# slimgroup/SetIntersectionProjection.jl

Measured on AMD Instinct MI355X. Metric: PARSDMM iterations/sec, higher is better.
Workload: dtype f32

## Files before the change

### setintersectionprojection.jl_amd/csrc/kernels_cds.hip

```cpp
#include <cstdlib>
#include <stdexcept>
#include <string>

#include "sipx_device.h"
#define SIPX_CG_GRID launch_blocks(3)
#ifndef SIPX_F64_VEC
#define SIPX_F64_VEC 2
#endif

namespace sipx {

template <typename T, int V>
struct LoadStored {
  const T* __restrict__ x;
  __device__ __forceinline__ Vec<T, V> operator()(long long c) const { return ldv_u<T, V>(x + c); }
};
template <typename T, int V>
struct LoadFused {
  const T* __restrict__ r;
  const T* __restrict__ p;
  T beta;
  __device__ __forceinline__ Vec<T, V> operator()(long long c) const {
    const Vec<T, V> rv = ldv_u<T, V>(r + c), pv = ldv_u<T, V>(p + c);
    Vec<T, V> o;
#pragma unroll
    for (int k = 0; k < V; ++k) o.v[k] = rv.v[k] + beta * pv.v[k];
    return o;
  }
};

template <typename T, int V, int D, typename XL>
__device__ __forceinline__ void cds_rows(long long N, const T* __restrict__ R, const CdsArgs& a, const XL& xl, long long r,
                                         T (&acc)[V]) {
  const int d = D ? D : a.d;
#pragma unroll
  for (int k = 0; k < V; ++k) acc[k] = T(0);
  if constexpr (D > 0) {
    Vec<T, V> rv[D], xv[D];
#pragma unroll
    for (int b = 0; b < D; ++b) {
      if (a.sym) {
        rv[b] = a.off[b] >= 0 ? ldv<T, V>(R + (long long)b * N + r)
                              : ldv_u<T, V>(R + (long long)a.partner[b] * N + r + a.off[b]);
      } else {
        rv[b] = ldv_nt<T, V>(R + (long long)b * N + r);
      }
      xv[b] = xl(r + a.off[b]);
    }
#pragma unroll
    for (int b = 0; b < D; ++b) {
      const long long c = r + a.off[b];
#pragma unroll
      for (int k = 0; k < V; ++k) {
        const T t = acc[k] + rv[b].v[k] * xv[b].v[k];
        acc[k] = (c + k >= 0 && c + k < N) ? t : acc[k];
      }
    }
  } else {
    for (int b = 0; b < d; ++b) {
      const long long c = r + a.off[b];
      const Vec<T, V> rv = !a.sym ? ldv_nt<T, V>(R + (long long)b * N + r)
                                  : (a.off[b] >= 0 ? ldv<T, V>(R + (long long)b * N + r)
                                                   : ldv_u<T, V>(R + (long long)a.partner[b] * N + c));
      const Vec<T, V> xv = xl(c);
#pragma unroll
      for (int k = 0; k < V; ++k) {
        const T t = acc[k] + rv.v[k] * xv.v[k];
        acc[k] = (c + k >= 0 && c + k < N) ? t : acc[k];
      }
    }
  }
}

template <typename T, int V, int D, int MODE>
__global__ __launch_bounds__(BLOCK) void k_cds(long long N, long long r0, long long r1, const T* __restrict__ R, CdsArgs a,
                                               const T* __restrict__ x, T* __restrict__ y, const T* __restrict__ b,
                                               T* __restrict__ pout, T* __restrict__ xold, double* __restrict__ partials,
                                               const int* __restrict__ done) {
  if (MODE == 1 && *done) return;
  const long long nvec = r1 / V;
  double acc0 = 0, acc1 = 0;
  for (long long vi = r0 / V + (long long)blockIdx.x * BLOCK + threadIdx.x; vi < nvec; vi += (long long)gridDim.x * BLOCK) {
    const long long r = vi * V;
    T s[V];
    cds_rows<T, V, D>(N, R, a, LoadStored<T, V>{x}, r, s);
    if (MODE == 0) {
      Vec<T, V> o;
#pragma unroll
      for (int k = 0; k < V; ++k) o.v[k] = s[k];
      stv_nt<T, V>(y + r, o);
    } else if (MODE == 1) {
      const Vec<T, V> pv = ldv<T, V>(x + r);
      Vec<T, V> o;
#pragma unroll
      for (int k = 0; k < V; ++k) {
        o.v[k] = s[k];
        acc0 += (double)pv.v[k] * (double)s[k];
      }
      stv_nt<T, V>(y + r, o);
    } else {
      const Vec<T, V> bv = ldv<T, V>(b + r);
      const Vec<T, V> xv = ldv<T, V>(x + r);
      Vec<T, V> o;
#pragma unroll
      for (int k = 0; k < V; ++k) {
        o.v[k] = bv.v[k] - s[k];
        acc0 += (double)o.v[k] * (double)o.v[k];
        acc1 += (double)bv.v[k] * (double)bv.v[k];
      }
      stv<T, V>(y + r, o);
      if (pout) stv<T, V>(pout + r, o);
      if (xold) stv<T, V>(xold + r, xv);
    }
  }
  if (MODE == 1) {
    double acc[1] = {acc0};
    block_reduce_store<1>(acc, partials, 0);
  } else if (MODE == 2) {
    double acc[2] = {acc0, acc1};
    block_reduce_store<2>(acc, partials, 0);
  }
}

constexpr int march_role(int ord, int b) {
  constexpr int o1[7] = {0, 1, 2, 3, 4, 5, 6}, o2[7] = {0, 5, 3, 1, 2, 4, 6};
  return ord == 1 ? o1[b] : o2[b];
}
template <typename T>
__device__ __forceinline__ T ata_value(const Grid& G, int nblk, const int* dir, const T* ihs, long long o, const Coord& c) {
  T val = (nblk == 0 && o == 0) ? T(1) : T(0);
  for (int q = 0; q < nblk; ++q) {
    const int d = dir[q];
    const T ih = ihs[q], nih = -ih;
    const int cc = coord_of(c, d);
    const long long st = G.st[d];
    if (o == 0) {
      if (cc > 0) val = val + ih * ih;
      if (cc < G.n[d] - 1) val = val + nih * nih;
    } else if (o == st) {
      if (cc < G.n[d] - 1) val = val + nih * ih;
    } else if (o == -st) {
      if (cc > 0) val = val + ih * nih;
    }
  }
  return val;
}

constexpr int QP_MAXB = 9, QP_MAXT = 8, QP_TAB = 160;
struct QPlanTerm {
  int kind;
  int nblk;
  int dir[3];
  int tab;
};
template <typename T>
struct QPlan {
  int nbands;
  int col[QP_MAXB], nterms[QP_MAXB];
  QPlanTerm t[QP_MAXB][QP_MAXT];
  int ntab;
  T tab[QP_TAB];
};

struct NoExtra {};
template <typename T>
struct QTab {
  const T* tab;
};
template <typename X>
struct IsQTab { static constexpr bool value = false; };
template <typename T>
struct IsQTab<QTab<T>> { static constexpr bool value = true; };
template <typename T>
__device__ __forceinline__ void load_class_tab(const QTab<T>& u, T* tab) {
  for (int i = threadIdx.x; i < QT_N; i += blockDim.x) tab[i] = u.tab[i];
}
template <typename X, typename T>
__device__ __forceinline__ void load_class_tab(const X&, T*) {}
__device__ __forceinline__ int line_class(long long c, long long n) { return c == 0 ? 0 : (c == n - 1 ? 2 : 1); }
template <typename T, int V>
__device__ __forceinline__ Vec<T, V> tab_row(const T* tab, int role, int cyz, long long i0, long long n1) {
  const T* e = tab + 27 * role + cyz;
  const T first = e[0], mid = e[1], last = e[2];
  Vec<T, V> v;
#pragma unroll
  for (int k = 0; k < V; ++k) v.v[k] = i0 + k == 0 ? first : (i0 + k == n1 - 1 ? last : mid);
  return v;
}
__device__ __forceinline__ void publish_ticket(unsigned long long* ticket, unsigned seq, int iter, int done);
constexpr int MARCH_NT = 512;
template <typename T, int V, int ORD, int MODE, typename X>
__global__ __launch_bounds__(MARCH_NT) void k_cds_march(long long n1, long long n2, long long n3, long long z0, long long z1, const T* __restrict__ R0,
                                                        const T* __restrict__ R1, const T* __restrict__ R2, const T* __restrict__ R3,
                                                        const T* __restrict__ x, T* __restrict__ y, const T* __restrict__ b,
                                                        T* __restrict__ pout, T* __restrict__ xold, double* __restrict__ partials,
                                                        const int* __restrict__ done, int lgLX, int tiles_x, int tiles_y, int zchunk,
                                                        long long items, CgState<T>* __restrict__ st, CgState<T>* __restrict__ host,
                                                        unsigned long long* ticket, X extra) {
  constexpr bool TAB = IsQTab<X>::value;
  if (MODE == 1 && *done) return;
  T beta = T(0);
  if (MODE == 3) {
    if (st->done) return;
    const double ss = block_sum_partials_n<MARCH_NT>(partials + NB);
    const T rr = (T)ss;
    const T res = (T)sqrt(ss) / st->nr0;
    const bool conv = res <= st->tol;
    beta = rr / st->gamma;
    if (blockIdx.x == 0 && threadIdx.x == 0) {
      st->ss = ss;
      st->res_last = res;
      if (conv) { st->flag = 0; st->done = 1; } else { st->beta = beta; }
      st->rr = rr;
      *host = *st;
      publish_ticket(ticket, st->seq, st->iters, conv ? 1 : 0);
    }
    if (conv) return;
  }
  auto ldx = [&](long long at) -> Vec<T, V> {
    Vec<T, V> v = ldv<T, V>(x + at);
    if (MODE == 3) {
      const Vec<T, V> pv = ldv<T, V>(b + at);
#pragma unroll
      for (int k = 0; k < V; ++k) v.v[k] = v.v[k] + beta * pv.v[k];
    }
    return v;
  };
  auto ldx1 = [&](long long at) -> T { return MODE == 3 ? x[at] + beta * b[at] : x[at]; };
  __shared__ T sx[2][V][MARCH_NT], sr[TAB ? 1 : 2][TAB ? 1 : V][TAB ? 1 : MARCH_NT];
  __shared__ T ctab[TAB ? QT_N : 1];
  if (TAB) {
    load_class_tab(extra, ctab);
    __syncthreads();
  }
  const int tid = threadIdx.x, LX = 1 << lgLX, tx = tid & (LX - 1), ty = tid >> lgLX, TY = MARCH_NT >> lgLX;
  const long long st1 = n1, st2 = n1 * n2, N = st2 * n3;
  const long long tiles = (long long)tiles_x * tiles_y;
  double acc0 = 0, acc1 = 0;
  for (long long item = blockIdx.x; item < items; item += gridDim.x) {
    const long long zc = item / tiles, tile = item - zc * tiles;
    const int tile_y = (int)(tile / tiles_x), tile_x = (int)(tile - (long long)tile_y * tiles_x);
    const long long i0 = ((long long)tile_x * LX + tx) * V, j = (long long)tile_y * TY + ty;
    const bool active = i0 < n1 && j < n2;
    const long long k0 = z0 + zc * zchunk, k1 = (k0 + zchunk < z1) ? k0 + zchunk : z1;
    const unsigned go = active ? (unsigned)(i0 + st1 * j) : 0u;
    __syncthreads();
    Vec<T, V> xm = zerov<T, V>(), x0 = zerov<T, V>(), rzm = zerov<T, V>();
    if (active) {
      xm = ldx(st2 * (k0 - 1) + go);
      x0 = ldx(st2 * k0 + go);
      if (k0 > 0 && TAB) {
        rzm = tab_row<T, V>(ctab, 3, 3 * line_class(j, n2) + 9 * line_class(k0 - 1, n3), i0, n1);
      } else if (k0 > 0) {
        rzm = ldv<T, V>(R3 + st2 * (k0 - 1) + go);
      }
    }
    for (long long kz = k0; kz < k1; ++kz) {
      const int par = (int)(kz & 1);
      const long long pz = st2 * kz;
      Vec<T, V> xp = zerov<T, V>(), r0 = xp, r1 = xp, r2 = xp, r3 = xp, bv = xp;
      const int cz = TAB ? line_class(kz, n3) : 0, cyz = TAB ? 3 * line_class(j, n2) + 9 * cz : 0;
      const int cyz_up = !TAB ? 0 : (j > 0 ? 3 * line_class(j - 1, n2) + 9 * cz : 3 * line_class(n2 - 1, n2) + 9 * line_class(kz - 1, n3));
      if (active) {
        xp = ldx(pz + st2 + go);
        if constexpr (TAB) {
          r0 = tab_row<T, V>(ctab, 0, cyz, i0, n1);
          r1 = tab_row<T, V>(ctab, 1, cyz, i0, n1);
          r2 = tab_row<T, V>(ctab, 2, cyz, i0, n1);
          r3 = tab_row<T, V>(ctab, 3, cyz, i0, n1);
        } else {
          r0 = ldv_nt<T, V>(R0 + pz + go);
          r1 = ldv_nt<T, V>(R1 + pz + go);
          r2 = ldv_nt<T, V>(R2 + pz + go);
          r3 = ldv_nt<T, V>(R3 + pz + go);
        }
        if (MODE == 2) bv = ldv<T, V>(b + pz + go);
      }
#pragma unroll
      for (int k = 0; k < V; ++k) {
        sx[par][k][tid] = x0.v[k];
        if constexpr (!TAB) sr[par][k][tid] = r2.v[k];
      }
      T xl = __shfl_up(x0.v[V - 1], 1, 64), xr = __shfl_down(x0.v[0], 1, 64), rl = TAB ? T(0) : __shfl_up(r1.v[V - 1], 1, 64);
      const long long r = pz + go;
      if (TAB && r > 0)
        rl = i0 > 0 ? ctab[27 + line_class(i0 - 1, n1) + cyz] : ctab[27 + line_class(n1 - 1, n1) + cyz_up];
      if (active) {
        if (tx == 0 || (tid & 63) == 0) {
          xl = ldx1(r - 1);
          if (!TAB) rl = r > 0 ? R1[r - 1] : T(0);
        }
        if (tx == LX - 1 || (tid & 63) == 63) xr = ldx1(r + V);
      }
      __syncthreads();
      if (active) {
        Vec<T, V> xu = zerov<T, V>(), xd = xu, ru = xu;
        if (TAB && r - st1 >= 0) ru = tab_row<T, V>(ctab, 2, cyz_up, i0, n1);
        if (ty > 0) {
#pragma unroll
          for (int k = 0; k < V; ++k) {
            xu.v[k] = sx[par][k][tid - LX];
            if constexpr (!TAB) ru.v[k] = sr[par][k][tid - LX];
          }
        } else {
          xu = ldx(r - st1);
          if (!TAB && r - st1 >= 0) ru = ldv<T, V>(R2 + r - st1);
        }
        if (ty < TY - 1 && j + 1 < n2) {
#pragma unroll
          for (int k = 0; k < V; ++k) xd.v[k] = sx[par][k][tid + LX];
        } else {
          xd = ldx(r + st1);
        }
        const bool up = r >= st1, down = r + st1 < N, below = r >= st2, above = r + st2 < N, first = r == 0, last = r + V == N;
        Vec<T, V> o4;
#pragma unroll
        for (int k = 0; k < V; ++k) {
          const T rv[7] = {r0.v[k], k == 0 ? rl : r1.v[k - 1], r1.v[k], ru.v[k], r2.v[k], rzm.v[k], r3.v[k]};
          const T xv[7] = {x0.v[k], k == 0 ? xl : x0.v[k - 1], k == V - 1 ? xr : x0.v[k + 1], xu.v[k], xd.v[k], xm.v[k], xp.v[k]};
          const bool in[7] = {true, k > 0 || !first, k < V - 1 || !last, up, down, below, above};
          T acc = T(0);
#pragma unroll
          for (int q = 0; q < 7; ++q) {
            const int role = march_role(ORD, q);
            const T t = acc + rv[role] * xv[role];
            acc = in[role] ? t : acc;
          }
          o4.v[k] = acc;
        }
        if (MODE == 0) {
          stv_nt<T, V>(y + r, o4);
        } else if (MODE == 1 || MODE == 3) {
#pragma unroll
          for (int k = 0; k < V; ++k) acc0 += (double)x0.v[k] * (double)o4.v[k];
          stv_nt<T, V>(y + r, o4);
          if (MODE == 3) stv<T, V>(pout + r, x0);
        } else {
          Vec<T, V> o;
#pragma unroll
          for (int k = 0; k < V; ++k) {
            o.v[k] = bv.v[k] - o4.v[k];
            acc0 += (double)o.v[k] * (double)o.v[k];
            acc1 += (double)bv.v[k] * (double)bv.v[k];
          }
          stv<T, V>(y + r, o);
          if (pout) stv<T, V>(pout + r, o);
          if (xold) stv<T, V>(xold + r, x0);
        }
      }
      xm = x0; x0 = xp; rzm = r3;
    }
  }
  if (MODE != 0) {
    __shared__ double sm[2][MARCH_NT / 64];
    const double v0 = wave_sum(acc0), v1 = wave_sum(acc1);
    __syncthreads();
    if ((tid & 63) == 0) { sm[0][tid >> 6] = v0; sm[1][tid >> 6] = v1; }
    __syncthreads();
    if (tid < (MODE == 2 ? 2 : 1)) {
      double s = 0;
#pragma unroll
      for (int i = 0; i < MARCH_NT / 64; ++i) s += sm[tid][i];
      double* row = partials + (long long)tid * NB;
      row[blockIdx.x] = s;
      for (int jj = blockIdx.x + gridDim.x; jj < NB; jj += gridDim.x) row[jj] = 0.0;
    }
  }
}

struct MarchGeom {
  int lg, tiles_x, tiles_y, zchunk, grid;
  long long items;
};
template <typename T>
static bool march_geom(long long N, long long r0, long long r1, const CdsArgs& a, MarchGeom& m) {
  const int sw = env_knobs().cds_march;
  const long long zc_env = env_knobs().cds_march_zchunk;
  if (sw == 0 || !a.march || !a.sym || a.d != 7) return false;
  constexpr int V = sizeof(T) == 8 ? 2 : 4;
  const long long n1 = a.gn[0], n2 = a.gn[1], n3 = a.gn[2], st2 = n1 * n2;
  if (n1 % V != 0 || n1 * n2 * n3 != N || r0 % st2 != 0 || r1 % st2 != 0 || r1 <= r0) return false;
  const long long nvx = n1 / V;
  int lg = 0;
  while ((1 << lg) < nvx && lg < 6) ++lg;
  const int LX = 1 << lg, TY = MARCH_NT / LX;
  const int tiles_x = (int)((nvx + LX - 1) / LX), tiles_y = (int)((n2 + TY - 1) / TY);
  const long long tiles = (long long)tiles_x * tiles_y, planes = (r1 - r0) / st2;
  long long zchunk = planes * tiles / 2048;
  if (zchunk < 16) zchunk = 16;
  if (sw == 2 && zc_env > 0) zchunk = zc_env;
  if (zchunk > planes) zchunk = planes;
  const long long nchunks = (planes + zchunk - 1) / zchunk, items = tiles * nchunks;
  if (items < 384 && sw != 2) return false;
  m = MarchGeom{lg, tiles_x, tiles_y, (int)zchunk, (int)(items < NB ? items : NB), items};
  return true;
}
template <typename T>
bool K<T>::march_applies(long long N, const CdsArgs& a) {
  MarchGeom m;
  return march_geom<T>(N, 0, N, a, m);
}

template <typename T, int MODE>
static bool try_march(hipStream_t s, long long N, long long r0, long long r1, const T* R, const CdsArgs& a, const T* x, T* y, const T* b,
                      T* pout, T* xold, double* partials, const int* done, CgState<T>* st = nullptr, CgState<T>* host = nullptr,
                      unsigned long long* ticket = nullptr) {
  MarchGeom m;
  if (!march_geom<T>(N, r0, r1, a, m)) return false;
  constexpr int V = sizeof(T) == 8 ? 2 : 4;
  const long long n1 = a.gn[0], n2 = a.gn[1], n3 = a.gn[2], st2 = n1 * n2;
  const T *R0 = R + (long long)a.mb[0] * N, *R1 = R + (long long)a.mb[1] * N, *R2 = R + (long long)a.mb[2] * N, *R3 = R + (long long)a.mb[3] * N;
#define SIPX_MARCH(ORD, XT, XV)                                                                                                      \
  hipLaunchKernelGGL((k_cds_march<T, V, ORD, MODE, XT>), dim3(m.grid), dim3(MARCH_NT), 0, s, n1, n2, n3, r0 / st2, r1 / st2, R0, R1, R2, R3, x, y, b, \
                     pout, xold, partials, done, m.lg, m.tiles_x, m.tiles_y, m.zchunk, m.items, st, host, ticket, XV)
  if (a.qtab) {
    const QTab<T> tab{(const T*)a.qtab};
    if (a.march == 1) SIPX_MARCH(1, QTab<T>, tab);
    else SIPX_MARCH(2, QTab<T>, tab);
  } else if (a.march == 1) {
    SIPX_MARCH(1, NoExtra, NoExtra{});
  } else {
    SIPX_MARCH(2, NoExtra, NoExtra{});
  }
#undef SIPX_MARCH
  return true;
}

template <typename T, int MODE>
static void launch_cds(hipStream_t s, long long N, long long r0, long long r1, const T* R, const CdsArgs& a, const T* x, T* y,
                       const T* b, T* pout, T* xold, double* partials, const int* done) {
  if (a.d < 1 || a.d > MAXD) throw std::runtime_error("cds: band count out of range");
  if (r0 < 0 || r1 > N || r0 > r1) throw std::runtime_error("cds: row range outside the matrix");
  int read_bands = a.d;
  if (a.sym) { read_bands = 0; for (int b = 0; b < a.d; ++b) read_bands += a.off[b] >= 0 ? 1 : 0; }
  if (a.qtab) read_bands = 0;
  const double rw = (double)(r1 - r0) * sizeof(T), extra = MODE == 2 ? 4.0 : 2.0;
  const double moved_extra = (MODE == 2 && !xold) ? 3.0 : extra;
  ObsScope obs(MODE == 0 ? KID_CDS_SPMV : (MODE == 1 ? KID_CDS_DOT : KID_CDS_RESID), s, (a.d + extra) * rw, (read_bands + moved_extra) * rw);
  if (try_march<T, MODE>(s, N, r0, r1, R, a, x, y, b, pout, xold, partials, done)) {
    SIPX_HIP(hipGetLastError());
    return;
  }
  if (a.qtab) throw std::runtime_error("internal: Q's class table is in use but the z-marching product does not apply");
#define SIPX_CDS(V, D) \
  hipLaunchKernelGGL((k_cds<T, V, D, MODE>), dim3(fit_grid((r1 - r0) / V, SIPX_CG_GRID)), dim3(BLOCK), 0, s, N, r0, r1, R, a, x, y, b, pout, xold, partials, done)
  constexpr int VW = sizeof(T) == 8 ? SIPX_F64_VEC : 4;
  if (N % 4 == 0 && r0 % 4 == 0 && r1 % 4 == 0) {
    switch (a.d) {
      case 1: SIPX_CDS(VW, 1); break;
      case 3: SIPX_CDS(VW, 3); break;
      case 5: SIPX_CDS(VW, 5); break;
      case 7: SIPX_CDS(VW, 7); break;
      default: SIPX_CDS(VW, 0); break;
    }
  } else {
    SIPX_CDS(1, 0);
  }
#undef SIPX_CDS
  SIPX_HIP(hipGetLastError());
}

template <typename T>
void K<T>::spmv(hipStream_t s, const Grid&, long long N, const T* R, const CdsArgs& a, const T* x, T* y) {
  launch_cds<T, 0>(s, N, 0, N, R, a, x, y, nullptr, nullptr, nullptr, nullptr, nullptr);
}
template <typename T>
void K<T>::spmv_dot(hipStream_t s, long long N, long long r0, long long r1, const T* R, const CdsArgs& a, const T* p, T* Ap,
                    double* partials, const CgState<T>* st) {
  launch_cds<T, 1>(s, N, r0, r1, R, a, p, Ap, nullptr, nullptr, nullptr, partials, &st->done);
}
template <typename T>
void K<T>::resid(hipStream_t s, long long N, long long r0, long long r1, const T* R, const CdsArgs& a, const T* x, const T* b,
                 T* r, T* p, T* xold, double* partials) {
  launch_cds<T, 2>(s, N, r0, r1, R, a, x, r, b, p, xold, partials, nullptr);
}

template <typename T, int V>
__device__ __forceinline__ void stencil_rows(const Grid& G, const StencilQ<T>& q, const T* __restrict__ x, long long g,
                                             const Vec<T, V>& xc, T (&acc)[V]) {
  const Coord c = coords(G, g);
#pragma unroll
  for (int k = 0; k < V; ++k) acc[k] = q.w0 * xc.v[k];
#pragma unroll
  for (int dir = 0; dir < 3; ++dir) {
    if (!(q.mask & (1 << dir))) continue;
    const long long st = G.st[dir];
    const int nd = (int)G.n[dir], cd = coord_of(c, dir);
    const Vec<T, V> xm = ldv_u<T, V>(x + g - st), xp = ldv_u<T, V>(x + g + st);
#pragma unroll
    for (int k = 0; k < V; ++k) {
      const int ck = cd + (dir == 0 ? k : 0);
      const T a = xc.v[k] - xm.v[k], b = xc.v[k] - xp.v[k];
      const T t = (ck > 0 ? a : T(0)) + (ck < nd - 1 ? b : T(0));
      acc[k] = acc[k] + q.w[dir] * t;
    }
  }
}

template <typename T, int V, int MODE>
__global__ __launch_bounds__(BLOCK) void k_sq(Grid G, StencilQ<T> q, const T* __restrict__ x, T* __restrict__ y,
                                              const T* __restrict__ b, T* __restrict__ pout, T* __restrict__ xold,
                                              double* __restrict__ partials, const int* __restrict__ done) {
  if (MODE == 1 && *done) return;
  const long long nvec = G.N / V;
  double acc0 = 0, acc1 = 0;
  for (long long vi = (long long)blockIdx.x * BLOCK + threadIdx.x; vi < nvec; vi += (long long)gridDim.x * BLOCK) {
    const long long r = vi * V;
    const Vec<T, V> xv = ldv<T, V>(x + r);
    T s[V];
    stencil_rows<T, V>(G, q, x, r, xv, s);
    Vec<T, V> o;
    if (MODE == 0) {
#pragma unroll
      for (int k = 0; k < V; ++k) o.v[k] = s[k];
      stv_nt<T, V>(y + r, o);
    } else if (MODE == 1) {
#pragma unroll
      for (int k = 0; k < V; ++k) {
        o.v[k] = s[k];
        acc0 += (double)xv.v[k] * (double)s[k];
      }
      stv_nt<T, V>(y + r, o);
    } else {
      const Vec<T, V> bv = ldv<T, V>(b + r);
#pragma unroll
      for (int k = 0; k < V; ++k) {
        o.v[k] = bv.v[k] - s[k];
        acc0 += (double)o.v[k] * (double)o.v[k];
        acc1 += (double)bv.v[k] * (double)bv.v[k];
      }
      stv<T, V>(y + r, o);
      if (pout) stv<T, V>(pout + r, o);
      if (xold) stv<T, V>(xold + r, xv);
    }
  }
  if (MODE == 1) {
    double acc[1] = {acc0};
    block_reduce_store<1>(acc, partials, 0);
  } else if (MODE == 2) {
    double acc[2] = {acc0, acc1};
    block_reduce_store<2>(acc, partials, 0);
  }
}

template <typename T, int MODE>
static void launch_sq(hipStream_t s, const Grid& G, const StencilQ<T>& q, const T* x, T* y, const T* b, T* pout, T* xold,
                      double* partials, const int* done) {
  ObsScope obs(MODE == 0 ? KID_SQ_SPMV : (MODE == 1 ? KID_SQ_DOT : KID_SQ_RESID), s, (MODE == 2 ? 4.0 : 2.0) * (double)G.N * sizeof(T));
  if (G.N % 4 == 0 && G.n[0] % 4 == 0)
    hipLaunchKernelGGL((k_sq<T, 4, MODE>), dim3(NB_7), dim3(BLOCK), 0, s, G, q, x, y, b, pout, xold, partials, done);
  else
    hipLaunchKernelGGL((k_sq<T, 1, MODE>), dim3(NB_7), dim3(BLOCK), 0, s, G, q, x, y, b, pout, xold, partials, done);
  SIPX_HIP(hipGetLastError());
}
template <typename T>
void K<T>::sq_spmv(hipStream_t s, const Grid& G, const StencilQ<T>& q, const T* x, T* y) {
  launch_sq<T, 0>(s, G, q, x, y, nullptr, nullptr, nullptr, nullptr, nullptr);
}
template <typename T>
void K<T>::sq_spmv_dot(hipStream_t s, const Grid& G, const StencilQ<T>& q, const T* p, T* Ap, double* partials,
                       const CgState<T>* st) {
  launch_sq<T, 1>(s, G, q, p, Ap, nullptr, nullptr, nullptr, partials, &st->done);
}
template <typename T>
void K<T>::sq_resid(hipStream_t s, const Grid& G, const StencilQ<T>& q, const T* x, const T* b, T* r, T* p, T* xold,
                    double* partials) {
  launch_sq<T, 2>(s, G, q, x, r, b, p, xold, partials, nullptr);
}

template <typename T, int V>
__global__ __launch_bounds__(BLOCK) void k_q_axpy(long long N, T* __restrict__ q, const T* __restrict__ a, T alpha) {
  const long long nvec = N / V;
  for (long long vi = (long long)blockIdx.x * BLOCK + threadIdx.x; vi < nvec; vi += (long long)gridDim.x * BLOCK) {
    Vec<T, V> qv = ldv<T, V>(q + vi * V);
    const Vec<T, V> av = ldv<T, V>(a + vi * V);
#pragma unroll
    for (int k = 0; k < V; ++k) qv.v[k] = qv.v[k] + alpha * av.v[k];
    stv<T, V>(q + vi * V, qv);
  }
}
template <typename T>
void K<T>::q_axpy(hipStream_t s, long long N, T* Qband, const T* Aband, T alpha) {
  if (N % 4 == 0)
    hipLaunchKernelGGL((k_q_axpy<T, 4>), dim3(NB), dim3(BLOCK), 0, s, N, Qband, Aband, alpha);
  else
    hipLaunchKernelGGL((k_q_axpy<T, 1>), dim3(NB), dim3(BLOCK), 0, s, N, Qband, Aband, alpha);
  SIPX_HIP(hipGetLastError());
}

struct GenArgs {
  int nblk;
  int dir[3];
  int nband;
  long long off[7];
};
template <typename T>
__global__ __launch_bounds__(BLOCK) void k_gen_ata(Grid G, GenArgs a, T ih0, T ih1, T ih2, T* __restrict__ R) {
  const T ihs[3] = {ih0, ih1, ih2};
  for (long long g = (long long)blockIdx.x * BLOCK + threadIdx.x; g < G.N; g += (long long)gridDim.x * BLOCK) {
    const Coord c = coords(G, g);
    for (int b = 0; b < a.nband; ++b) R[(long long)b * G.N + g] = ata_value<T>(G, a.nblk, a.dir, ihs, a.off[b], c);
  }
}

template <typename T, int V>
__global__ __launch_bounds__(BLOCK) void k_q_update(Grid G, long long r0, long long r1, CdsArgs q, QArgs<T> a, T* __restrict__ Q) {
  const long long nvec = r1 / V;
  for (long long vi = r0 / V + (long long)blockIdx.x * BLOCK + threadIdx.x; vi < nvec; vi += (long long)gridDim.x * BLOCK) {
    const long long g = vi * V;
    Coord c[V];
#pragma unroll
    for (int k = 0; k < V; ++k) { c[k] = coords(G, g); c[k].i += k; }
    for (int b = 0; b < q.d; ++b) {
      const long long o = q.off[b];
      if (q.sym && o < 0) continue;
      bool touched = false;
      Vec<T, V> qv;
      for (int si = 0; si < a.nsets; ++si) {
        const QSet<T>& S = a.s[si];
        int j = -1;
        for (int t = 0; t < S.nband; ++t) if (S.off[t] == o) j = t;
        if (j < 0) continue;
        if (!touched) { qv = ldv<T, V>(Q + (long long)b * G.N + g); touched = true; }
        if (S.ata) {
          const Vec<T, V> av = ldv_nt<T, V>(S.ata + (long long)j * G.N + g);
#pragma unroll
          for (int k = 0; k < V; ++k) qv.v[k] = qv.v[k] + S.alpha * av.v[k];
        } else {
#pragma unroll
          for (int k = 0; k < V; ++k) qv.v[k] = qv.v[k] + S.alpha * ata_value<T>(G, S.nblk, S.dir, S.ih, o, c[k]);
        }
      }
      if (touched) stv<T, V>(Q + (long long)b * G.N + g, qv);
    }
  }
}

template <typename T, int V>
__global__ __launch_bounds__(BLOCK) void k_q_update_plan(Grid G, long long r0, long long r1, QPlan<T> p, T* __restrict__ Q) {
  __shared__ T tab[QP_TAB];
  for (int i = threadIdx.x; i < p.ntab; i += BLOCK) tab[i] = p.tab[i];
  __syncthreads();
  const int n1 = (int)G.n[0], n2 = (int)G.n[1], n3 = (int)G.n[2];
  const long long nvec = r1 / V;
  for (long long vi = r0 / V + (long long)blockIdx.x * BLOCK + threadIdx.x; vi < nvec; vi += (long long)gridDim.x * BLOCK) {
    const long long g = vi * V;
    const Coord c = coords(G, g);
    int cx[V];
#pragma unroll
    for (int k = 0; k < V; ++k) cx[k] = (c.i + k) == 0 ? 0 : ((c.i + k) == n1 - 1 ? 2 : 1);
    const int cy = c.j == 0 ? 0 : (c.j == n2 - 1 ? 2 : 1), cz = c.k == 0 ? 0 : (c.k == n3 - 1 ? 2 : 1);
    for (int b = 0; b < p.nbands; ++b) {
      T* row = Q + (long long)p.col[b] * G.N + g;
      Vec<T, V> qv = ldv<T, V>(row);
      for (int ti = 0; ti < p.nterms[b]; ++ti) {
        const QPlanTerm& t = p.t[b][ti];
        if (t.kind == 0) {
          const T v = tab[t.tab];
#pragma unroll
          for (int k = 0; k < V; ++k) qv.v[k] = qv.v[k] + v;
        } else if (t.kind == 1) {
          int base = 0, mulx = 0, m3 = 1;
          for (int q = 0; q < t.nblk; ++q) {
            const int d = t.dir[q];
            if (d == 0) mulx += m3; else base += (d == 1 ? cy : cz) * m3;
            m3 *= 3;
          }
#pragma unroll
          for (int k = 0; k < V; ++k) qv.v[k] = qv.v[k] + tab[t.tab + base + mulx * cx[k]];
        } else {
          const int d = t.dir[0];
          const int edge = t.kind == 2 ? 2 : 0;
          const T on = tab[t.tab], off = tab[t.tab + 1];
#pragma unroll
          for (int k = 0; k < V; ++k) {
            const int cl = d == 0 ? cx[k] : (d == 1 ? cy : cz);
            qv.v[k] = qv.v[k] + (cl != edge ? on : off);
          }
        }
      }
      stv<T, V>(row, qv);
    }
  }
}
// ... 574 lines not shown
```

Before: 898.0.

## Software-pipeline next-plane loads in CDS march stencil kernel

Restructures the z-marching stencil loop so that the next plane's x, halo-edge and side loads are issued one iteration ahead and drained with an explicit s_waitcnt before the stores. Edge loads for the up, down and left/right neighbours are merged into a single precomputed offset per thread, and the pipeline depth is chosen at compile time per mode and table variant. The intent is to hide global-memory latency behind the stencil arithmetic. In exchange it raises register pressure, which the occupancy hint of 4 blocks per CU in launch_bounds may force into spills, and it adds a 32-bit offset guard on the geometry.

Measured after the change: 906.4 (median of 6 runs). Within noise of the previous version (+0.9%).

```diff
diff --git a/setintersectionprojection.jl_amd/csrc/kernels_cds.hip b/setintersectionprojection.jl_amd/csrc/kernels_cds.hip
--- a/setintersectionprojection.jl_amd/csrc/kernels_cds.hip
+++ b/setintersectionprojection.jl_amd/csrc/kernels_cds.hip
@@ -190,7 +190,7 @@
 __device__ __forceinline__ void publish_ticket(unsigned long long* ticket, unsigned seq, int iter, int done);
 constexpr int MARCH_NT = 512;
 template <typename T, int V, int ORD, int MODE, typename X>
-__global__ __launch_bounds__(MARCH_NT) void k_cds_march(long long n1, long long n2, long long n3, long long z0, long long z1, const T* __restrict__ R0,
+__global__ __launch_bounds__(MARCH_NT, 4) void k_cds_march(long long n1, long long n2, long long n3, long long z0, long long z1, const T* __restrict__ R0,
                                                         const T* __restrict__ R1, const T* __restrict__ R2, const T* __restrict__ R3,
                                                         const T* __restrict__ x, T* __restrict__ y, const T* __restrict__ b,
                                                         T* __restrict__ pout, T* __restrict__ xold, double* __restrict__ partials,
@@ -198,6 +198,8 @@
                                                         long long items, CgState<T>* __restrict__ st, CgState<T>* __restrict__ host,
                                                         unsigned long long* ticket, X extra) {
   constexpr bool TAB = IsQTab<X>::value;
+  constexpr int DEPTH = TAB ? ((MODE != 3 || sizeof(T) == 4) ? 2 : 1) : (MODE < 2 ? 2 : 0);
+  constexpr bool AHEAD = DEPTH == 2;
   if (MODE == 1 && *done) return;
   T beta = T(0);
   if (MODE == 3) {
@@ -217,16 +219,49 @@
     }
     if (conv) return;
   }
-  auto ldx = [&](long long at) -> Vec<T, V> {
-    Vec<T, V> v = ldv<T, V>(x + at);
-    if (MODE == 3) {
-      const Vec<T, V> pv = ldv<T, V>(b + at);
-#pragma unroll
-      for (int k = 0; k < V; ++k) v.v[k] = v.v[k] + beta * pv.v[k];
-    }
+  struct XRaw { Vec<T, V> a, b; };
+  struct XRaw1 { T a, b; };
+  struct PlaneRaw {
+    XRaw xp, e;
+    XRaw1 s;
+    Vec<T, V> bv;
+  };
+  struct PlaneIn {
+    Vec<T, V> xp, e;
+    T s;
+    Vec<T, V> bv;
+  };
+  auto ldraw = [&](long long at) -> XRaw {
+    XRaw v;
+    v.a = ldv<T, V>(x + at);
+    v.b = MODE == 3 ? ldv<T, V>(b + at) : zerov<T, V>();
     return v;
   };
-  auto ldx1 = [&](long long at) -> T { return MODE == 3 ? x[at] + beta * b[at] : x[at]; };
+  auto ldraw1 = [&](long long at) -> XRaw1 { return XRaw1{x[at], MODE == 3 ? b[at] : T(0)}; };
+  auto value = [&](const XRaw& w) -> Vec<T, V> {
+    Vec<T, V> v = w.a;
+    if (MODE == 3) {
+#pragma unroll
+      for (int k = 0; k < V; ++k) v.v[k] = v.v[k] + beta * w.b.v[k];
+    }
+    return v;
+  };
+  auto value1 = [&](const XRaw1& w) -> T { return MODE == 3 ? w.a + beta * w.b : w.a; };
+  auto ldx = [&](long long at) -> Vec<T, V> { return value(ldraw(at)); };
+  auto wait_loads = [] { __builtin_amdgcn_s_waitcnt(0x0F70); };
+  auto late = [&](long long at) -> Vec<T, V> {
+    const XRaw w = ldraw(at);
+    wait_loads();
+    return value(w);
+  };
+  auto late1 = [&](long long at) -> T {
+    const XRaw1 w = ldraw1(at);
+    wait_loads();
+    return value1(w);
+  };
+  auto values = [&](const PlaneRaw& w) -> PlaneIn { return PlaneIn{value(w.xp), value(w.e), value1(w.s), w.bv}; };
+  const XRaw zraw{zerov<T, V>(), zerov<T, V>()};
+  const PlaneRaw zplane{zraw, zraw, XRaw1{T(0), T(0)}, zerov<T, V>()};
   __shared__ T sx[2][V][MARCH_NT], sr[TAB ? 1 : 2][TAB ? 1 : V][TAB ? 1 : MARCH_NT];
   __shared__ T ctab[TAB ? QT_N : 1];
   if (TAB) {
@@ -236,6 +271,7 @@
   const int tid = threadIdx.x, LX = 1 << lgLX, tx = tid & (LX - 1), ty = tid >> lgLX, TY = MARCH_NT >> lgLX;
   const long long st1 = n1, st2 = n1 * n2, N = st2 * n3;
   const long long tiles = (long long)tiles_x * tiles_y;
+  __builtin_assume((n1 & (V - 1)) == 0);
   double acc0 = 0, acc1 = 0;
   for (long long item = blockIdx.x; item < items; item += gridDim.x) {
     const long long zc = item / tiles, tile = item - zc * tiles;
@@ -255,14 +291,31 @@
         rzm = ldv<T, V>(R3 + st2 * (k0 - 1) + go);
       }
     }
+    const bool from_up = ty == 0, from_down = !(ty < TY - 1 && j + 1 < n2), from_both = from_up && from_down;
+    const bool lane_l = tx == 0 || (tid & 63) == 0, lane_r = tx == LX - 1 || (tid & 63) == 63;
+    const unsigned geo = from_up ? go : go + 2u * (unsigned)st1, gso = lane_l ? go : go + (unsigned)V + 1u;
+    auto issue = [&](long long kz, bool inner, bool edge) -> PlaneRaw {
+      const long long pl = st2 * kz;
+      PlaneRaw w = zplane;
+      if (inner) w.xp = ldraw(pl + st2 + go);
+      if (edge && (from_up || from_down)) w.e = ldraw(pl - st1 + geo);
+      if (edge && (lane_l || lane_r)) w.s = ldraw1(pl - 1 + gso);
+      if (inner && MODE == 2) w.bv = ldv<T, V>(b + pl + go);
+      return w;
+    };
+    PlaneIn in = values(zplane);
+    if (AHEAD && active) in = values(issue(k0, true, true));
     for (long long kz = k0; kz < k1; ++kz) {
       const int par = (int)(kz & 1);
       const long long pz = st2 * kz;
-      Vec<T, V> xp = zerov<T, V>(), r0 = xp, r1 = xp, r2 = xp, r3 = xp, bv = xp;
+      Vec<T, V> r0 = zerov<T, V>(), r1 = r0, r2 = r0, r3 = r0;
       const int cz = TAB ? line_class(kz, n3) : 0, cyz = TAB ? 3 * line_class(j, n2) + 9 * cz : 0;
       const int cyz_up = !TAB ? 0 : (j > 0 ? 3 * line_class(j - 1, n2) + 9 * cz : 3 * line_class(n2 - 1, n2) + 9 * line_class(kz - 1, n3));
+      const long long r = pz + go;
+      Vec<T, V> rue = zerov<T, V>();
+      T rle = T(0);
+      PlaneRaw nxt = zplane;
       if (active) {
-        xp = ldx(pz + st2 + go);
         if constexpr (TAB) {
           r0 = tab_row<T, V>(ctab, 0, cyz, i0, n1);
           r1 = tab_row<T, V>(ctab, 1, cyz, i0, n1);
@@ -273,8 +326,14 @@
           r1 = ldv_nt<T, V>(R1 + pz + go);
           r2 = ldv_nt<T, V>(R2 + pz + go);
           r3 = ldv_nt<T, V>(R3 + pz + go);
+          if (from_up && r - st1 >= 0) rue = ldv<T, V>(R2 + r - st1);
+          if (lane_l && r > 0) rle = R1[r - 1];
         }
-        if (MODE == 2) bv = ldv<T, V>(b + pz + go);
+        if constexpr (AHEAD) {
+          if (kz + 1 < k1) nxt = issue(kz + 1, true, true);
+        } else {
+          in = values(issue(kz, true, DEPTH == 1));
+        }
       }
 #pragma unroll
       for (int k = 0; k < V; ++k) {
@@ -282,69 +341,76 @@
         if constexpr (!TAB) sr[par][k][tid] = r2.v[k];
       }
       T xl = __shfl_up(x0.v[V - 1], 1, 64), xr = __shfl_down(x0.v[0], 1, 64), rl = TAB ? T(0) : __shfl_up(r1.v[V - 1], 1, 64);
-      const long long r = pz + go;
       if (TAB && r > 0)
         rl = i0 > 0 ? ctab[27 + line_class(i0 - 1, n1) + cyz] : ctab[27 + line_class(n1 - 1, n1) + cyz_up];
+      __syncthreads();
+      const Vec<T, V> xp = in.xp, bv = in.bv;
+      Vec<T, V> o4 = zerov<T, V>();
       if (active) {
-        if (tx == 0 || (tid & 63) == 0) {
-          xl = ldx1(r - 1);
-          if (!TAB) rl = r > 0 ? R1[r - 1] : T(0);
+        if constexpr (DEPTH == 0) {
+          const PlaneIn late = values(issue(kz, false, true));
+          in.e = late.e;
+          in.s = late.s;
         }
-        if (tx == LX - 1 || (tid & 63) == 63) xr = ldx1(r + V);
-      }
-      __syncthreads();
-      if (active) {
+        if (lane_l) {
+          xl = in.s;
+          if (!TAB) rl = rle;
+        }
+        if (lane_r) xr = lane_l ? late1(r + V) : in.s;
         Vec<T, V> xu = zerov<T, V>(), xd = xu, ru = xu;
         if (TAB && r - st1 >= 0) ru = tab_row<T, V>(ctab, 2, cyz_up, i0, n1);
-        if (ty > 0) {
+        if (!from_up) {
 #pragma unroll
           for (int k = 0; k < V; ++k) {
             xu.v[k] = sx[par][k][tid - LX];
             if constexpr (!TAB) ru.v[k] = sr[par][k][tid - LX];
           }
         } else {
-          xu = ldx(r - st1);
-          if (!TAB && r - st1 >= 0) ru = ldv<T, V>(R2 + r - st1);
+          xu = in.e;
+          if (!TAB) ru = rue;
         }
-        if (ty < TY - 1 && j + 1 < n2) {
+        if (!from_down) {
 #pragma unroll
           for (int k = 0; k < V; ++k) xd.v[k] = sx[par][k][tid + LX];
         } else {
-          xd = ldx(r + st1);
+          xd = from_both ? late(r + st1) : in.e;
         }
         const bool up = r >= st1, down = r + st1 < N, below = r >= st2, above = r + st2 < N, first = r == 0, last = r + V == N;
-        Vec<T, V> o4;
 #pragma unroll
         for (int k = 0; k < V; ++k) {
           const T rv[7] = {r0.v[k], k == 0 ? rl : r1.v[k - 1], r1.v[k], ru.v[k], r2.v[k], rzm.v[k], r3.v[k]};
           const T xv[7] = {x0.v[k], k == 0 ? xl : x0.v[k - 1], k == V - 1 ? xr : x0.v[k + 1], xu.v[k], xd.v[k], xm.v[k], xp.v[k]};
-          const bool in[7] = {true, k > 0 || !first, k < V - 1 || !last, up, down, below, above};
+          const bool inside[7] = {true, k > 0 || !first, k < V - 1 || !last, up, down, below, above};
           T acc = T(0);
 #pragma unroll
           for (int q = 0; q < 7; ++q) {
             const int role = march_role(ORD, q);
             const T t = acc + rv[role] * xv[role];
-            acc = in[role] ? t : acc;
+            acc = inside[role] ? t : acc;
           }
           o4.v[k] = acc;
         }
-        if (MODE == 0) {
-          stv_nt<T, V>(y + r, o4);
-        } else if (MODE == 1 || MODE == 3) {
+        if (MODE == 1 || MODE == 3) {
 #pragma unroll
           for (int k = 0; k < V; ++k) acc0 += (double)x0.v[k] * (double)o4.v[k];
+        } else if (MODE == 2) {
+#pragma unroll
+          for (int k = 0; k < V; ++k) {
+            o4.v[k] = bv.v[k] - o4.v[k];
+            acc0 += (double)o4.v[k] * (double)o4.v[k];
+            acc1 += (double)bv.v[k] * (double)bv.v[k];
+          }
+        }
+      }
+      if constexpr (AHEAD) wait_loads();
+      if (active) {
+        if constexpr (AHEAD) in = values(nxt);
+        if (MODE == 0 || MODE == 1 || MODE == 3) {
           stv_nt<T, V>(y + r, o4);
           if (MODE == 3) stv<T, V>(pout + r, x0);
         } else {
-          Vec<T, V> o;
-#pragma unroll
-          for (int k = 0; k < V; ++k) {
-            o.v[k] = bv.v[k] - o4.v[k];
-            acc0 += (double)o.v[k] * (double)o.v[k];
-            acc1 += (double)bv.v[k] * (double)bv.v[k];
-          }
-          stv<T, V>(y + r, o);
-          if (pout) stv<T, V>(pout + r, o);
+          stv<T, V>(y + r, o4);
+          if (pout) stv<T, V>(pout + r, o4);
           if (xold) stv<T, V>(xold + r, x0);
         }
       }
@@ -380,6 +446,7 @@
   constexpr int V = sizeof(T) == 8 ? 2 : 4;
   const long long n1 = a.gn[0], n2 = a.gn[1], n3 = a.gn[2], st2 = n1 * n2;
   if (n1 % V != 0 || n1 * n2 * n3 != N || r0 % st2 != 0 || r1 % st2 != 0 || r1 <= r0) return false;
+  if (st2 + 2 * n1 + V >= (1ll << 32)) return false;
   const long long nvx = n1 / V;
   int lg = 0;
   while ((1 << lg) < nvx && lg < 6) ++lg;
```
